# interaction-lab-uh/STROTSS-tensorflow

Measured on AMD Instinct MI355X. Metric: optimisation_steps_per_sec_1024px_pair, higher is better.
Workload: dtype f32; 1 GPU; 1024px content/style pair, 1024x1024 scale of the coarse-to-fine pyramid, 1024 samples x D=2179, VGG16 (seeded He-normal weights), RMSprop pixel update; scale_px=1024, samples=1024, parallelism=single GPU, tap_adjoint=deterministic (planned, sorted scatter)

## Files before the change

strotss-tensorflow_amd/csrc/gemm.hip:

```cpp
#include <stdlib.h>

#include "internal.h"
#include "mfma_pipe.h"
#include "mfma_x3.h"

namespace {

template <int BM, int BN, bool AKC, bool BKC>
__device__ __forceinline__ void gemm_mainloop(const float* __restrict__ A, int lda, int M,
                                              const float* __restrict__ B, int ldb, int N, int K,
                                              int m0, int n0, float* ldsA, float* ldsB,
                                              f32x16 (&acc)[BM / 64][BN / 64]) {
  f32x4 ra[BM / 32], rb[BN / 32];
  auto load = [&](int k0) {
    if constexpr (AKC) gload_kc<BM>(ra, A, lda, m0, M, k0); else gload_rc<BM>(ra, A, lda, m0, M, k0);
    if constexpr (BKC) gload_kc<BN>(rb, B, ldb, n0, N, k0); else gload_rc<BN>(rb, B, ldb, n0, N, k0);
  };
  load(0);
  for (int k0 = 0; k0 < K; k0 += 32) {
    __syncthreads();
    if constexpr (AKC) lds_store_kc<BM>(ldsA, ra); else lds_store_rc<BM>(ldsA, ra);
    if constexpr (BKC) lds_store_kc<BN>(ldsB, rb); else lds_store_rc<BN>(ldsB, rb);
    __syncthreads();
    if (k0 + 32 < K) load(k0 + 32);
// ... 224 lines not shown
  }
  return v;
}

template <int BM, int BN, class Epi>
int launch_pipe(const float* A, int lda, int M, long long strideA, const float* B, int ldb, int N,
                long long strideB, int K, int batch, Epi epi, hipStream_t s) {
  dim3 grid((unsigned)cdiv(N, BN) * cdiv(M, BM) * batch);
  if constexpr (BM == 128) {
    if (gemm_waves() == 8) {
      using Cfg = PipeCfg<BM, BN, (BN == 128 ? 2 : 4), (BN == 128 ? 4 : 2)>;
      hipLaunchKernelGGL((gemm_kc_pipe_kernel<Cfg, Epi>), grid, dim3(Cfg::NT), 0, s, A, lda, M, strideA, B, ldb, N,
                         strideB, K, epi);
      ST_LAUNCH_RET();
    }
  }
  {
    using Cfg = PipeCfg<BM, BN, 2, 2>;
    hipLaunchKernelGGL((gemm_kc_pipe_kernel<Cfg, Epi>), grid, dim3(Cfg::NT), 0, s, A, lda, M, strideA, B, ldb, N,
                       strideB, K, epi);
  }
  ST_LAUNCH_RET();
}

template <int BM, int BN, bool AKC, bool BKC, class Epi>
int launch(const float* A, int lda, int M, const float* B, int ldb, int N, int K, Epi epi,
           hipStream_t s) {
  dim3 grid(cdiv(N, BN), cdiv(M, BM));
  hipLaunchKernelGGL((gemm_kernel<BM, BN, AKC, BKC, Epi>), grid, dim3(256), 0, s, A, lda, M, B, ldb, N,
                     K, epi);
  ST_LAUNCH_RET();
}

}

int st_cosine_distance(const float* x, const float* rx, int nx, const float* y, const float* ry, int ny,
                       int ld, float* C, int ldc, hipStream_t s) {
  EpiCosDist e{rx, ry, C, ldc, nx, ny, (x == y && rx == ry && nx == ny) ? 1 : 0};
  return launch_pipe<64, 64>(x, ld, nx, 0, y, ld, ny, 0, ld, 1, e, s);
}

int st_l2_distance(const float* x, const float* xs, int nx, const float* y, const float* ys, int ny, int ld, int d,
                   float* C, int ldc, hipStream_t s) {
  EpiL2Dist e{xs, ys, C, ldc, nx, ny, (float)d};
  return launch_pipe<64, 64>(x, ld, nx, 0, y, ld, ny, 0, ld, 1, e, s);
}

int st_remd_cost(const float* x, const float* rx, const float* sx, int nx, const float* y, const float* ry, const float* sy,
                 int ny, int ld, int d, int metric, float* C, float* S, int ldc, hipStream_t s) {
  EpiRemdCost e{rx, ry, sx, sy, C, S, ldc, nx, ny, (float)d, metric};
  return launch_pipe<64, 64>(x, ld, nx, 0, y, ld, ny, 0, ld, 1, e, s);
}

int st_gram_tn(const float* A, int krows, int ld, float alpha, float* C, hipStream_t s) {
  EpiScaleStore e{C, ld, ld, ld, alpha, 0};
  return launch<64, 64, false, false>(A, ld, ld, A, ld, ld, krows, e, s);
}

int st_moment_fwd_gemm(const float* cy, int krows, int ld, const float* Sx, float* T, float inv_n,
                       float* partial, int* n_partial, hipStream_t s) {
  EpiMomentFwd e{Sx, T, ld, ld, ld, inv_n, partial};
  *n_partial = cdiv(ld, 64) * cdiv(ld, 64);
  return launch<64, 64, false, false>(cy, ld, ld, cy, ld, ld, krows, e, s);
}

int st_moment_bwd_gemm(const float* cy, int n, int ld, const float* T, float alpha, const float* bias,
                       float bias_scale, float* dY, hipStream_t s) {
  EpiAxpbyBias e{dY, ld, n, ld, alpha, bias, bias_scale};
  return launch_pipe<64, 64>(cy, ld, n, 0, T, ld, ld, 0, ld, 1, e, s);
}

int st_selfsim_bwd_gemm(const float* Mq, int ldm, int kpad, const float* bmat, const float* x, const float* r,
                        const float* q, int n, int ld, float g, float* dx, hipStream_t s) {
  EpiSelfsimBwd e{x, r, q, dx, ld, n, ld, g};
  return launch<64, 64, true, false>(Mq, ldm, n, bmat, ld, ld, kpad, e, s);
}

int st_gemm_nt_batched(const float* A, int lda, long long strideA, const float* B, int ldb, long long strideB,
                       float* C, int ldc, long long strideC, int M, int N, int K, int batch, hipStream_t s) {
  EpiScaleStore e{C, ldc, M, N, 1.0f, strideC};
  const long long t128 = (long long)cdiv(M, 128) * cdiv(N, 128);
  if (t128 * batch >= 512 && N % 128 == 0) {
    static int split = -1;
    if (split < 0) { const char* env = getenv("STROTSS_GEMM_TAIL_SPLIT"); split = env ? atoi(env) : 1; }
    const long long slots = 512, total = t128 * batch;
    const long long rem = total % slots;
    if (split && total > slots && rem != 0 && rem * 2 <= slots && slots % t128 == 0) {
      const int tail = (int)(rem / t128), head = batch - tail;
      int rc = launch_pipe<128, 128>(A, lda, M, strideA, B, ldb, N, strideB, K, head, e, s);
      if (rc != 0) return rc;
      EpiScaleStore e2{C + (long long)head * strideC, ldc, M, N, 1.0f, strideC};
      return launch_pipe<128, 64>(A + (long long)head * strideA, lda, M, strideA, B + (long long)head * strideB, ldb, N,
                                  strideB, K, tail, e2, s);
    }
    return launch_pipe<128, 128>(A, lda, M, strideA, B, ldb, N, strideB, K, batch, e, s);
  }
  const long long t64 = (long long)cdiv(M, 128) * cdiv(N, 64);
  if (t64 * batch >= 512) {
    static int split = -1;
    if (split < 0) { const char* env = getenv("STROTSS_GEMM_TAIL_SPLIT"); split = env ? atoi(env) : 1; }
    const long long slots = 512, total = t64 * batch, rem = total % slots;
    if (split && total > slots && rem != 0 && rem * 2 <= slots && slots % t64 == 0) {
      const int tail = (int)(rem / t64), head = batch - tail;
      int rc = launch_pipe<128, 64>(A, lda, M, strideA, B, ldb, N, strideB, K, head, e, s);
      if (rc != 0) return rc;
      EpiScaleStore e2{C + (long long)head * strideC, ldc, M, N, 1.0f, strideC};
      return launch_pipe<64, 64>(A + (long long)head * strideA, lda, M, strideA, B + (long long)head * strideB, ldb, N,
                                 strideB, K, tail, e2, s);
    }
    return launch_pipe<128, 64>(A, lda, M, strideA, B, ldb, N, strideB, K, batch, e, s);
  }
  return launch_pipe<64, 64>(A, lda, M, strideA, B, ldb, N, strideB, K, batch, e, s);
}

int st_x3_split_rows(const float* x, int rows, int ld, int K, long long stride_in, void* panels, int batch,
                     hipStream_t s) {
  const size_t total = (size_t)rows * (K >> 2);
  hipLaunchKernelGGL(x3_split_rows_kernel, dim3((unsigned)min((size_t)2048, (total + 255) / 256), batch), dim3(256), 0, s,
                     x, rows, ld, K, stride_in, (__bf16*)panels, (long long)3 * rows * K);
  ST_LAUNCH_RET();
}

struct EpiScaleStoreX3 : EpiScaleStore, X3NoPrefetch<EpiScaleStoreX3> {
  using EpiScaleStore::apply;
  using X3NoPrefetch<EpiScaleStoreX3>::apply;
};
struct X3NoMirror {
  template <class Epi, class Pre, class Acc, class Map>
  __device__ __forceinline__ void operator()(const Epi&, Pre&, float*, int, int, int, int, Acc&, const Map&) const {}
};
template <class Cfg>
struct X3Mirror {
  template <class Epi, class Pre, class Acc, class Map>
  __device__ __forceinline__ void operator()(const Epi& epi, Pre&, float* tile, int m0, int n0, int M, int N, Acc& acc,
                                             const Map& map) const {
    mirror_tile<Cfg::BM, Cfg::BN, Cfg::NT, true>(epi, tile, m0, n0, M, N, [&](auto put) {
#pragma unroll
      for (int im = 0; im < Cfg::T; ++im)
#pragma unroll
        for (int in = 0; in < Cfg::T; ++in)
#pragma unroll
          for (int reg = 0; reg < 16; ++reg) {
            const int r = m0 + map.row(im, reg), c = n0 + map.colof(in);
            put(r, c, (r < M && c < N) ? epi.value(r, c, acc[im][in][reg]) : 0.f);
          }
    });
  }
};

static bool x3_k16_enabled() {
  static const bool k16 = [] { const char* v = getenv("STROTSS_X3_K16"); return !v || atoi(v) != 0; }();
  return k16;
}
int st_gemm_x3_batched(const void* A, const void* B, float* C, int ldc, long long strideC, int M, int N, int K,
                       int batch, hipStream_t s, long min_tiles128) {
  EpiScaleStoreX3 e{{C, ldc, M, N, 1.0f, strideC}, {}};
  if ((long)cdiv(N, 128) * cdiv(M, 128) * batch >= min_tiles128 && x3_k16_enabled()) {
    using Cfg = X3CfgK16<3>;
    dim3 grid((unsigned)cdiv(N, 128) * cdiv(M, 128) * batch);
    hipLaunchKernelGGL((gemm_x3_kernel<Cfg, EpiScaleStoreX3, X3NoMirror>), grid, dim3(Cfg::NT), 0, s, (const __bf16*)A, M,
                       (long long)3 * M * K, (const __bf16*)B, N, (long long)3 * N * K, K, e, X3NoMirror{});
  } else if ((long)cdiv(N, 128) * cdiv(M, 128) * batch >= min_tiles128) {
    using Cfg = X3Cfg<128>;
    dim3 grid((unsigned)cdiv(N, 128) * cdiv(M, 128) * batch);
    hipLaunchKernelGGL((gemm_x3_kernel<Cfg, EpiScaleStoreX3, X3NoMirror>), grid, dim3(Cfg::NT), 0, s, (const __bf16*)A, M,
                       (long long)3 * M * K, (const __bf16*)B, N, (long long)3 * N * K, K, e, X3NoMirror{});
  } else {
    using Cfg = X3Cfg<64>;
    dim3 grid((unsigned)cdiv(N, 64) * cdiv(M, 64) * batch);
    hipLaunchKernelGGL((gemm_x3_kernel<Cfg, EpiScaleStoreX3, X3NoMirror>), grid, dim3(Cfg::NT), 0, s, (const __bf16*)A, M,
                       (long long)3 * M * K, (const __bf16*)B, N, (long long)3 * N * K, K, e, X3NoMirror{});
  }
  ST_LAUNCH_RET();
}

bool st_gemm_x3_f32a_ok(int M, int N, int batch, long min_tiles128) {
  return (long)cdiv(N, 128) * cdiv(M, 128) * batch >= min_tiles128 && x3_k16_enabled();
}
int st_gemm_x3_batched_f32a(const float* A, const void* B, float* C, int ldc, long long strideC, int M, int N, int K,
                            int batch, hipStream_t s, long min_tiles128) {
  if (!st_gemm_x3_f32a_ok(M, N, batch, min_tiles128)) return STROTSS_EINVAL;
  EpiScaleStoreX3 e{{C, ldc, M, N, 1.0f, strideC}, {}};
  using Cfg = X3CfgK16<3, true>;
  dim3 grid((unsigned)cdiv(N, 128) * cdiv(M, 128) * batch);
  hipLaunchKernelGGL((gemm_x3_kernel<Cfg, EpiScaleStoreX3, X3NoMirror>), grid, dim3(Cfg::NT), 0, s, A, M, (long long)M * K,
                     (const __bf16*)B, N, (long long)3 * N * K, K, e, X3NoMirror{});
  ST_LAUNCH_RET();
}

struct EpiSelfsimBwdX3 : EpiSelfsimBwd {
  template <int T> struct Pre { float dx0[T][T][16], x0[T][T][16], ri[T][16], qi[T][16]; };
  template <class P> __device__ __forceinline__ void prefetch(P& p, int im, int in, int reg, int row, int c) const {
    const int rr = min(row, M - 1);
    const size_t o = (size_t)rr * ld + min(c, N - 1);
    p.dx0[im][in][reg] = dx[o];
    p.x0[im][in][reg] = x[o];
    if (in == 0) { p.ri[im][reg] = r[rr]; p.qi[im][reg] = q[rr]; }
  }
  template <class P> __device__ __forceinline__ float apply(P& p, int im, int in, int reg, int row, int c, float v) const {
    const float ri = p.ri[im][reg];
    const float out = p.dx0[im][in][reg] + g * ri * (v - p.x0[im][in][reg] * ri * p.qi[im][reg]);
    if (row < M && c < N) dx[(size_t)row * ld + c] = out;
    return 0.f;
  }
};
struct EpiAxpbyBiasX3 : EpiAxpbyBias {
  template <int T> struct Pre { float c0[T][T][16], b[T]; };
  template <class P> __device__ __forceinline__ void prefetch(P& p, int im, int in, int reg, int r, int c) const {
    p.c0[im][in][reg] = C[(size_t)min(r, M - 1) * ldc + min(c, N - 1)];
    if (im == 0 && reg == 0) p.b[in] = bias[min(c, N - 1)];
  }
  template <class P> __device__ __forceinline__ float apply(P& p, int im, int in, int reg, int r, int c, float v) const {
    const float out = p.c0[im][in][reg] + alpha * v + bias_scale * p.b[in];
    if (r < M && c < N) C[(size_t)r * ldc + c] = out;
    return 0.f;
  }
};
struct EpiMomentFwdX3 {
  static constexpr bool SYMM = true;
  static constexpr int symm = 1;
  const float* Sx; __bf16* Tp; int ld; int M, N; float inv_n; float* partial;
  unsigned first_block = 0;
  __device__ __forceinline__ void set_batch(int) {}
  template <int T> struct Pre { float sx[T][T][16]; };
  template <class P> __device__ __forceinline__ void prefetch(P& p, int im, int in, int reg, int r, int c) const {
    p.sx[im][in][reg] = Sx[(size_t)min(r, M - 1) * ld + min(c, N - 1)];
  }
  template <class P> __device__ __forceinline__ float apply(P& p, int im, int in, int reg, int r, int c, float v) const {
    const float a = fabsf(v * inv_n - p.sx[im][in][reg]);
    const float w = (r < M && c < N && r <= c) ? (r == c ? 1.f : 2.f) : 0.f;
    return w * a;
  }
  __device__ __forceinline__ void finish(float* red, float local) const {
    const float s = block_sum_256(local, red);
    if (threadIdx.x == 0) partial[blockIdx.x - first_block] = s;
  }
};
template <class Cfg>
struct X3MomentStore {
  template <class Pre, class Acc, class Map>
  __device__ __forceinline__ void operator()(const EpiMomentFwdX3& epi, Pre& pre, float* tile, int m0, int n0, int M, int N,
                                             Acc& acc, const Map& map) const {
    constexpr int B = Cfg::BM, LD = B + 1;
    __syncthreads();
#pragma unroll
    for (int im = 0; im < Cfg::T; ++im)
#pragma unroll
      for (int in = 0; in < Cfg::T; ++in)
#pragma unroll
        for (int reg = 0; reg < 16; ++reg) {
          const int r = map.row(im, reg), c = map.colof(in);
          tile[r * LD + c] = signf(acc[im][in][reg] * epi.inv_n - pre.sx[im][in][reg]);
        }
    __syncthreads();
    const bool diag = n0 == m0;
    if (diag) {
      for (int i = threadIdx.x; i < B * B; i += Cfg::NT) {
        const int r = i / B, c = i - r * B;
        if (r > c) tile[r * LD + c] = tile[c * LD + r];
      }
      __syncthreads();
    }
    auto put8 = [&](int row, int k0, const float (&v)[8]) {
      bf16x8 o;
#pragma unroll
      for (int q = 0; q < 8; ++q) o[q] = (__bf16)v[q];
      *reinterpret_cast<bf16x8*>(epi.Tp + ((size_t)(k0 >> 5) * epi.ld + row) * 32 + (k0 & 31)) = o;
    };
    for (int i = threadIdx.x; i < B * (B / 8); i += Cfg::NT) {
      const int r = i / (B / 8), c8 = (i - r * (B / 8)) * 8;
      if (m0 + r >= M || n0 + c8 >= N) continue;
      float v[8];
#pragma unroll
      for (int q = 0; q < 8; ++q) v[q] = tile[r * LD + c8 + q];
      put8(m0 + r, n0 + c8, v);
    }
    if (!diag) {
      for (int i = threadIdx.x; i < B * (B / 8); i += Cfg::NT) {
        const int c = i % B, r8 = (i / B) * 8;
        if (n0 + c >= N || m0 + r8 >= M) continue;
        float v[8];
#pragma unroll
        for (int q = 0; q < 8; ++q) v[q] = tile[(r8 + q) * LD + c];
        put8(n0 + c, m0 + r8, v);
      }
    }
  }
};

struct EpiSymScaleX3 : X3NoPrefetch<EpiSymScaleX3> {
  using X3NoPrefetch<EpiSymScaleX3>::apply;
  static constexpr bool SYMM = true;
  static constexpr int symm = 1;
  float* C; int ld; int M, N; float alpha;
  __device__ __forceinline__ void set_batch(int) {}
  __device__ __forceinline__ float value(int, int, float v) const { return alpha * v; }
  __device__ __forceinline__ float apply(int r, int c, float v) const {
    if (r < M && c < N && r <= c) C[(size_t)r * ld + c] = alpha * v;
    return 0.f;
  }
  __device__ __forceinline__ void mirror(int r, int c, float val) const { C[(size_t)r * ld + c] = val; }
  __device__ __forceinline__ void finish(float*, float) const {}
};
int st_gram_tn_x3(const void* Pt, int npad, int ld, float alpha, float* C, hipStream_t s) {
  using Cfg = X3CfgK16<3>;
  EpiSymScaleX3 e{{}, C, ld, ld, ld, alpha};
  const int g = cdiv(ld, 128);
  hipLaunchKernelGGL((gemm_x3_kernel<Cfg, EpiSymScaleX3, X3Mirror<Cfg>>), dim3(g * (g + 1) / 2), dim3(Cfg::NT), 0, s,
                     (const __bf16*)Pt, ld, 0LL, (const __bf16*)Pt, ld, 0LL, npad, e, X3Mirror<Cfg>{});
  ST_LAUNCH_RET();
}

int st_moment_fwd_x3(const void* Pt, int npad, int ld, const float* Sx, void* Tp, float inv_n, float* partial,
                     int* n_partial, hipStream_t s) {
  using Cfg = X3CfgK16<3>;
  EpiMomentFwdX3 e{Sx, (__bf16*)Tp, ld, ld, ld, inv_n, partial, 0u};
  const int g = cdiv(ld, 128);
  *n_partial = g * (g + 1) / 2;
  hipLaunchKernelGGL((gemm_x3_kernel<Cfg, EpiMomentFwdX3, X3MomentStore<Cfg>>), dim3(g * (g + 1) / 2), dim3(Cfg::NT), 0, s,
                     (const __bf16*)Pt, ld, 0LL, (const __bf16*)Pt, ld, 0LL, npad, e, X3MomentStore<Cfg>{});
  ST_LAUNCH_RET();
}

int st_loss_forward_group_x3(const void* Pt, int npad, int ld, const float* Sx, void* Tp, float inv_n, float* partial,
                             int* n_partial,
                             const void* xp, const float* rp, int n, long long pstride, long long rstride, float* Dx,
                             int ldc, long long dstride,
                             const void* xs, const float* rs, int ns, float* Ct, int ldt, hipStream_t s) {
  using CM = X3CfgK16<3>;
  using CC = X3Cfg<64>;
  const unsigned gm = cdiv(ld, 128), nm = gm * (gm + 1) / 2;
  const unsigned g = cdiv(n, 64), nc = g * (g + 1) / 2 * 2;
  const unsigned gs = cdiv(ns, 64), nr = g * gs;
  *n_partial = (int)nm;
  X3Problem<EpiMomentFwdX3> p0{(const __bf16*)Pt, ld, 0LL, (const __bf16*)Pt, ld, 0LL, npad,
                               EpiMomentFwdX3{Sx, (__bf16*)Tp, ld, ld, ld, inv_n, partial, 0u}, 0, 0, nm};
  X3Problem<EpiCosDistX3> p1{(const __bf16*)xp, n, pstride, (const __bf16*)xp, n, pstride, ld,
                             EpiCosDistX3{{rp, rp, Dx, ldc, n, n, 1}, {}, rstride, dstride}, 0, 0, nc};
  int bh = 0, bw = 0;
// ... 118 lines not shown
```

strotss-tensorflow_amd/csrc/mfma_x3.h:

```cpp
#pragma once
#include <type_traits>

#include "mfma_pipe.h"

typedef __bf16 bf16x8 __attribute__((ext_vector_type(8)));
typedef __bf16 bf16x4 __attribute__((ext_vector_type(4)));
typedef unsigned int u32x4 __attribute__((ext_vector_type(4)));

struct Split3 { bf16x4 h, m, l; };
__device__ __forceinline__ Split3 split3(const f32x4 x) {
  Split3 s;
#pragma unroll
  for (int k = 0; k < 4; ++k) {
    const __bf16 h = (__bf16)x[k];
    const float r1 = x[k] - (float)h;
    const __bf16 m = (__bf16)r1;
    const float r2 = r1 - (float)m;
    s.h[k] = h; s.m[k] = m; s.l[k] = (__bf16)r2;
  }
  return s;
}

__host__ __device__ __forceinline__ size_t x3_panel_elems(size_t rows, size_t K) { return 3 * rows * K; }
__device__ __forceinline__ void x3_store4(__bf16* base, size_t rows, size_t row, int k0, const f32x4 v) {
  const Split3 s = split3(v);
  const size_t o = ((size_t)(k0 >> 5) * 3 * rows + row) * 32 + (k0 & 31);
  *reinterpret_cast<bf16x4*>(base + o) = s.h;
  *reinterpret_cast<bf16x4*>(base + o + rows * 32) = s.m;
  *reinterpret_cast<bf16x4*>(base + o + 2 * rows * 32) = s.l;
}

template <int B_, int NPB_ = 3>
struct X3Cfg {
  static_assert(B_ == 128 || B_ == 64, "x3 main loop: 128 x 128 or 64 x 64 tiles");
  static_assert(NPB_ == 3 || (NPB_ == 1 && B_ == 128), "single-plane B: 128 x 128 tiles only");
  static constexpr int NPB = NPB_, NPROD = NPB_ == 3 ? 6 : 3;
  static constexpr int BM = B_, BN = B_, WM = 2, WN = 2, NT = 256;
  static constexpr int T = B_ / 64;
  static constexpr int TM = T, TN = T;
  static constexpr int PL = B_ * 64;
  static constexpr int STAGE = (3 + NPB_) * PL;
  static constexpr int LDS_BYTES = 3 * STAGE;
  static constexpr int G = B_ / 64;
  static constexpr int NP = (3 + NPB_) * G;
  static constexpr bool K16 = false, AF32 = false;
};

#define X3_WAIT_VM(n) asm volatile("s_waitcnt vmcnt(" #n ")" ::: "memory")

template <int G, int NPL = 3>
struct X3Operand {
  const char* base;
  unsigned off[G];
  unsigned plane;
  unsigned cur;
  __device__ __forceinline__ X3Operand(const __bf16* p, int rows, int row0) {
    const int lane = threadIdx.x & 63, wave = __builtin_amdgcn_readfirstlane(threadIdx.x >> 6);
    base = reinterpret_cast<const char*>(p);
    plane = (unsigned)rows * 64u;
    cur = 0;
    const int chunk = (lane & 3) ^ ((lane >> 4) & 3);
#pragma unroll
    for (int g = 0; g < G; ++g) {
      const int row = min(row0 + (G * wave + g) * 16 + (lane >> 2), rows - 1);
      off[g] = (unsigned)row * 64u + (unsigned)chunk * 16u;
    }
  }
  __device__ __forceinline__ void dma(int pl, int g, unsigned char* lds_dst) const {
    const char* src = base + (size_t)(cur + pl * plane) + off[g];
    __builtin_amdgcn_global_load_lds((const __attribute__((address_space(1))) void*)src,
                                     (__attribute__((address_space(3))) void*)lds_dst, 16, 0, 0);
  }
  __device__ __forceinline__ void advance() { cur += NPL * plane; }
};

template <class Cfg>
__device__ __forceinline__ void x3_mainloop(unsigned char* lds, int steps, X3Operand<Cfg::G, 3>& oa,
                                            X3Operand<Cfg::G, Cfg::NPB>& ob, f32x16 (&acc)[Cfg::T][Cfg::T]) {
  constexpr int PL = Cfg::PL, STAGE = Cfg::STAGE, T = Cfg::T, G = Cfg::G, NP = Cfg::NP, HALF = Cfg::BM / 2;
  constexpr int NPB = Cfg::NPB, NPROD = Cfg::NPROD;
  const int t = threadIdx.x, lane = t & 63, wave = __builtin_amdgcn_readfirstlane(t >> 6);
  const int wm = wave >> 1, wn = wave & 1, l31 = lane & 31, hh = lane >> 5;
  auto dma_piece = [&](int j, unsigned char* stage) {
#ifdef X3_ABL_NO_DMA
    return;
#endif
    const int pl = j / G, g = j % G;
    unsigned char* dst = stage + pl * PL + (G * wave + g) * 1024;
    if (pl < 3) oa.dma(pl, g, dst); else ob.dma(pl - 3, g, dst);
  };
  auto dma_tile = [&](unsigned char* stage) {
#pragma unroll
    for (int j = 0; j < NP; ++j) dma_piece(j, stage);
    oa.advance(); ob.advance();
  };
  auto wait_one_tile_in_flight = [&]() {
    if constexpr (NP == 12) X3_WAIT_VM(12); else if constexpr (NP == 8) X3_WAIT_VM(8); else X3_WAIT_VM(6);
  };
  const int f = (l31 >> 2) & 3;
  const int a_rd = (wm * HALF + l31) * 64 + ((hh ^ f) << 4);
  const int b_rd = 3 * PL + (wn * HALF + l31) * 64 + ((hh ^ f) << 4);
  bf16x8 fa[2][3][T], fb[2][NPB][T];
  auto read_frags = [&](const unsigned char* stage, int kc, int slot) {
#ifdef X3_ABL_NO_FRAG
    if (stage != lds) return;
#endif
    const unsigned char* pa = stage + (a_rd ^ (kc << 5));
    const unsigned char* pb = stage + (b_rd ^ (kc << 5));
#pragma unroll
    for (int p = 0; p < 3; ++p) {
#pragma unroll
      for (int i = 0; i < T; ++i) {
        fa[slot][p][i] = *reinterpret_cast<const bf16x8*>(pa + p * PL + i * 2048);
        if (p < NPB) fb[slot][p][i] = *reinterpret_cast<const bf16x8*>(pb + p * PL + i * 2048);
      }
    }
  };
  constexpr int PA[6] = {2, NPB == 3 ? 0 : 1, NPB == 3 ? 1 : 0, 1, 0, 0};
  constexpr int PB[6] = {0, NPB == 3 ? 2 : 0, NPB == 3 ? 1 : 0, 0, 1, 0};
  constexpr int STRIDE = NPROD * T * T / NP;
  static_assert(STRIDE >= 1, "more DMA pieces than MFMAs in a k-chunk");

  unsigned char* s_cur = lds;
  unsigned char* s_nxt = lds + STAGE;
  unsigned char* s_nn = lds + 2 * STAGE;
  dma_tile(s_cur);
  if (steps > 1) { dma_tile(s_nxt); wait_one_tile_in_flight(); } else { X3_WAIT_VM(0); }
  __builtin_amdgcn_s_barrier();
  read_frags(s_cur, 0, 0);

  auto kstep = [&](auto mode_tag) {
    constexpr int MODE = decltype(mode_tag)::value;
#pragma unroll
    for (int c = 0; c < 2; ++c) {
#pragma unroll
      for (int q = 0; q < NPROD; ++q) {
        if (c == 0 && q == 1) {
          __builtin_amdgcn_sched_barrier(0);
          read_frags(s_cur, 1, 1);
          __builtin_amdgcn_sched_barrier(0);
        }
#pragma unroll
        for (int im = 0; im < T; ++im) {
#pragma unroll
          for (int in_ = 0; in_ < T; ++in_) {
#ifndef X3_ABL_NO_MFMA
            acc[im][in_] = __builtin_amdgcn_mfma_f32_32x32x16_bf16(fa[c][PA[q]][im], fb[c][PB[q]][in_], acc[im][in_], 0, 0, 0);
#else
            acc[im][in_][0] += (float)fa[c][PA[q]][im][0] + (float)fb[c][PB[q]][in_][0];
#endif
            const int done = (q * T + im) * T + in_ + 1;
            if (MODE == 2 && c == 0 && done % STRIDE == 0 && done / STRIDE <= NP) {
              __builtin_amdgcn_sched_barrier(0);
              dma_piece(done / STRIDE - 1, s_nn);
              __builtin_amdgcn_sched_barrier(0);
            }
          }
        }
        if (c == 1 && q == 0 && MODE != 0) {
          __builtin_amdgcn_sched_barrier(0);
          if (MODE == 2) wait_one_tile_in_flight(); else X3_WAIT_VM(0);
          asm volatile("s_waitcnt lgkmcnt(0)" ::: "memory");
#ifndef X3_ABL_NO_BARRIER
          __builtin_amdgcn_s_barrier();
#endif
          asm volatile("" ::: "memory");
          read_frags(s_nxt, 0, 0);
          __builtin_amdgcn_sched_barrier(0);
        }
      }
    }
    if (MODE == 2) { oa.advance(); ob.advance(); }
    unsigned char* tmp = s_cur; s_cur = s_nxt; s_nxt = s_nn; s_nn = tmp;
  };
  int s = 0;
  for (; s + 2 < steps; ++s) kstep(std::integral_constant<int, 2>{});
  if (steps > 1) kstep(std::integral_constant<int, 1>{});
  kstep(std::integral_constant<int, 0>{});
}

template <int NPB_ = 3, bool AF32_ = false, int WQ_ = AF32_ ? 1 : 3>
struct X3CfgK16 {
  static_assert(NPB_ == 3, "K16 ring: three B planes");
  static_assert(WQ_ >= 0 && WQ_ <= 4, "K16 ring: the wait needs at least one product group after it");
  static constexpr int NPB = NPB_, NPROD = 6;
  static constexpr bool AF32 = AF32_;
  static constexpr int WQ = WQ_;
  static constexpr int BM = 128, BN = 128, WM = 2, WN = 2, NT = 256;
  static constexpr int T = 2, TM = 2, TN = 2;
  static constexpr int PL = 128 * 32;
  static constexpr int NPA = AF32_ ? 2 : 3;
  static constexpr int ABYTES = NPA * PL;
  static constexpr int STAGE = ABYTES + 3 * PL;
  static constexpr int LDS_BYTES = 3 * STAGE;
  static constexpr int G = 1, NP = NPA + 3;
  static constexpr bool K16 = true;
};

struct X3OperandK16 {
  const char* base;
  unsigned off;
  unsigned plane;
  unsigned cur;
  __device__ __forceinline__ X3OperandK16(const __bf16* p, int rows, int row0) {
    const int lane = threadIdx.x & 63, wave = __builtin_amdgcn_readfirstlane(threadIdx.x >> 6);
    base = reinterpret_cast<const char*>(p);
    plane = (unsigned)rows * 64u;
    cur = 0;
    const int row = min(row0 + wave * 32 + (lane >> 1), rows - 1);
    off = (unsigned)row * 64u + (unsigned)((lane & 1) ^ ((lane >> 4) & 1)) * 16u;
  }
  __device__ __forceinline__ void dma(int pl, unsigned char* lds_dst) const {
    const char* src = base + (size_t)(cur + pl * plane) + off;
    __builtin_amdgcn_global_load_lds((const __attribute__((address_space(1))) void*)src,
                                     (__attribute__((address_space(3))) void*)lds_dst, 16, 0, 0);
  }
  __device__ __forceinline__ void advance(int half) { cur += half ? 3u * plane - 32u : 32u; }
};

struct X3OperandK16F32 {
  const char* base;
  unsigned off[2];
  unsigned kblk;
  unsigned cur;
  __device__ __forceinline__ X3OperandK16F32(const float* p, int rows, int row0) {
    const int lane = threadIdx.x & 63, wave = __builtin_amdgcn_readfirstlane(threadIdx.x >> 6);
    base = reinterpret_cast<const char*>(p);
    kblk = (unsigned)rows * 128u;
    cur = 0;
    const int chunk = (lane & 3) ^ ((lane >> 4) & 3);
#pragma unroll
    for (int g = 0; g < 2; ++g) {
      const int row = min(row0 + wave * 32 + g * 16 + (lane >> 2), rows - 1);
      off[g] = (unsigned)row * 128u + (unsigned)chunk * 16u;
    }
  }
  __device__ __forceinline__ void dma(int g, unsigned char* lds_dst) const {
    const char* src = base + (size_t)cur + off[g];
    __builtin_amdgcn_global_load_lds((const __attribute__((address_space(1))) void*)src,
                                     (__attribute__((address_space(3))) void*)lds_dst, 16, 0, 0);
  }
  __device__ __forceinline__ void advance(int half) { cur += half ? kblk - 64u : 64u; }
};

__device__ __forceinline__ void x3_f32_store4(float* base, size_t rows, size_t row, int k0, const f32x4 v) {
  *reinterpret_cast<f32x4*>(base + ((size_t)(k0 >> 5) * rows + row) * 32 + (k0 & 31)) = v;
}

__device__ __forceinline__ void x3_split8(const f32x4 lo, const f32x4 hi, bf16x8& h, bf16x8& m, bf16x8& l) {
  const Split3 a = split3(lo), b = split3(hi);
  h = __builtin_shufflevector(a.h, b.h, 0, 1, 2, 3, 4, 5, 6, 7);
  m = __builtin_shufflevector(a.m, b.m, 0, 1, 2, 3, 4, 5, 6, 7);
  l = __builtin_shufflevector(a.l, b.l, 0, 1, 2, 3, 4, 5, 6, 7);
}

template <class Cfg> struct X3Ops {
  using A = std::conditional_t<Cfg::K16, std::conditional_t<Cfg::AF32, X3OperandK16F32, X3OperandK16>, X3Operand<Cfg::G, 3>>;
  using B = std::conditional_t<Cfg::K16, X3OperandK16, X3Operand<Cfg::G, Cfg::NPB>>;
  using AT = std::conditional_t<Cfg::AF32, float, __bf16>;
};

template <class Cfg, class OA>
__device__ __forceinline__ void x3_k16_prologue(unsigned char* lds, OA& oa, X3OperandK16& ob) {
#ifndef X3_ABL_NO_DMA
  const int wave = __builtin_amdgcn_readfirstlane(threadIdx.x >> 6);
#pragma unroll
  for (int h = 0; h < 2; ++h) {
    unsigned char* stage = lds + h * Cfg::STAGE;
#pragma unroll
    for (int j = 0; j < Cfg::NP; ++j) {
      if (j >= Cfg::NPA) ob.dma(j - Cfg::NPA, stage + Cfg::ABYTES + (j - Cfg::NPA) * Cfg::PL + wave * 1024);
      else if constexpr (Cfg::AF32) oa.dma(j, stage + wave * 2048 + j * 1024);
      else oa.dma(j, stage + j * Cfg::PL + wave * 1024);
    }
    oa.advance(h); ob.advance(h);
  }
#endif
}

template <class Cfg, class OA>
__device__ __forceinline__ void x3_mainloop_k16(unsigned char* lds, int steps, OA& oa, X3OperandK16& ob,
                                                f32x16 (&acc)[2][2]) {
  constexpr int PL = Cfg::PL, STAGE = Cfg::STAGE, NPA = Cfg::NPA, NP = Cfg::NP, WQ = Cfg::WQ;
  constexpr bool AF32 = Cfg::AF32;
  static_assert(NP == 5 || NP == 6, "K16 ring: 5 or 6 DMA pieces per wave and step");
  const int t = threadIdx.x, lane = t & 63, wave = __builtin_amdgcn_readfirstlane(t >> 6);
  const int wm = wave >> 1, wn = wave & 1, l31 = lane & 31, hh = lane >> 5;
  auto dma_piece = [&](int j, unsigned char* stage) {
#ifdef X3_ABL_NO_DMA
    return;
#endif
    if (j >= NPA) ob.dma(j - NPA, stage + Cfg::ABYTES + (j - NPA) * PL + wave * 1024);
    else if constexpr (AF32) oa.dma(j, stage + wave * 2048 + j * 1024);
    else oa.dma(j, stage + j * PL + wave * 1024);
  };
  constexpr int IN_FLIGHT = 4 * (WQ + 1) < NP ? 4 * (WQ + 1) : NP;
  auto wait_next_tile = [&]() {
    if constexpr (IN_FLIGHT == 6) X3_WAIT_VM(6); else if constexpr (IN_FLIGHT == 5) X3_WAIT_VM(5); else X3_WAIT_VM(4);
  };
  int half = 0;
  const int sw = (hh ^ ((l31 >> 3) & 1)) << 4;
  const int a_rd = (wm * 64 + l31) * 32 + sw;
  const int b_rd = Cfg::ABYTES + (wn * 64 + l31) * 32 + sw;
  const int af = (l31 >> 2) & 3;
  const int a_rd0 = (wm * 64 + l31) * 64 + (((2 * hh) ^ af) << 4), a_rd1 = (wm * 64 + l31) * 64 + (((2 * hh + 1) ^ af) << 4);
  bf16x8 fa[2][3][2], fb[2][3][2];
  f32x4 ra[2][2];
  auto read_frags = [&](const unsigned char* stage, int slot) {
#ifdef X3_ABL_NO_FRAG
    if (stage != lds) return;
#endif
#pragma unroll
    for (int i = 0; i < 2; ++i) {
      if constexpr (AF32) {
        ra[i][0] = *reinterpret_cast<const f32x4*>(stage + a_rd0 + i * 2048);
        ra[i][1] = *reinterpret_cast<const f32x4*>(stage + a_rd1 + i * 2048);
      }
#pragma unroll
      for (int p = 0; p < 3; ++p) {
        if constexpr (!AF32) fa[slot][p][i] = *reinterpret_cast<const bf16x8*>(stage + a_rd + p * PL + i * 1024);
        fb[slot][p][i] = *reinterpret_cast<const bf16x8*>(stage + b_rd + p * PL + i * 1024);
      }
    }
  };
  auto split_a = [&](int slot) {
    if constexpr (AF32) {
#pragma unroll
      for (int i = 0; i < 2; ++i) x3_split8(ra[i][0], ra[i][1], fa[slot][0][i], fa[slot][1][i], fa[slot][2][i]);
    }
  };
  constexpr int PA[6] = {2, 0, 1, 1, 0, 0};
  constexpr int PB[6] = {0, 2, 1, 0, 1, 0};

  unsigned char* s_cur = lds;
  unsigned char* s_nxt = lds + STAGE;
  unsigned char* s_nn = lds + 2 * STAGE;
  if constexpr (NP == 6) X3_WAIT_VM(6); else X3_WAIT_VM(5);
  __builtin_amdgcn_s_barrier();
  read_frags(s_cur, 0);
  split_a(0);

  auto kstep = [&](auto mode_tag, auto slot_tag) {
    constexpr int MODE = decltype(mode_tag)::value, SLOT = decltype(slot_tag)::value;
#pragma unroll
    for (int q = 0; q < 6; ++q) {
#pragma unroll
      for (int im = 0; im < 2; ++im) {
#pragma unroll
        for (int in_ = 0; in_ < 2; ++in_) {
#ifndef X3_ABL_NO_MFMA
          acc[im][in_] = __builtin_amdgcn_mfma_f32_32x32x16_bf16(fa[SLOT][PA[q]][im], fb[SLOT][PB[q]][in_], acc[im][in_], 0, 0, 0);
#else
          acc[im][in_][0] += (float)fa[SLOT][PA[q]][im][0] + (float)fb[SLOT][PB[q]][in_][0];
#endif
          const int done = (q * 2 + im) * 2 + in_ + 1;
          if (MODE == 2 && done <= NP) {
            __builtin_amdgcn_sched_barrier(0);
            dma_piece(done - 1, s_nn);
            __builtin_amdgcn_sched_barrier(0);
          }
        }
      }
      if (q == WQ && MODE != 0) {
        __builtin_amdgcn_sched_barrier(0);
        if (MODE == 2) wait_next_tile(); else X3_WAIT_VM(0);
        asm volatile("s_waitcnt lgkmcnt(0)" ::: "memory");
#ifndef X3_ABL_NO_BARRIER
        __builtin_amdgcn_s_barrier();
#endif
        asm volatile("" ::: "memory");
        read_frags(s_nxt, SLOT ^ 1);
        __builtin_amdgcn_sched_barrier(0);
        split_a(SLOT ^ 1);
      }
    }
    if (MODE == 2) { oa.advance(half); ob.advance(half); half ^= 1; }
    unsigned char* tmp = s_cur; s_cur = s_nxt; s_nxt = s_nn; s_nn = tmp;
  };
  using I0 = std::integral_constant<int, 0>; using I1 = std::integral_constant<int, 1>; using I2 = std::integral_constant<int, 2>;
  int s = 0;
  for (; s + 3 < steps; s += 2) { kstep(I2{}, I0{}); kstep(I2{}, I1{}); }
  kstep(I1{}, I0{});
  kstep(I0{}, I1{});
}

template <class D>
struct X3NoPrefetch {
  template <int T> struct Pre {};
  template <class P> __device__ __forceinline__ void prefetch(P&, int, int, int, int, int) const {}
  template <class P> __device__ __forceinline__ float apply(P&, int, int, int, int r, int c, float v) const {
    return static_cast<const D*>(this)->apply(r, c, v);
  }
};

template <class Cfg, class Epi, class Mirror>
__device__ __forceinline__ void gemm_x3_tile(unsigned char* lds, unsigned bid, unsigned nblk,
                                             const typename X3Ops<Cfg>::AT* __restrict__ A, int M,
                                             long long strideA, const __bf16* __restrict__ B, int N, long long strideB, int K,
                                             const Epi& epi_in, const Mirror& mirror, int xbh, int xbw) {
  Epi epi = epi_in;
  const unsigned gx = (N + Cfg::BN - 1) / Cfg::BN, gy = (M + Cfg::BM - 1) / Cfg::BM;
  unsigned tile = xcd_swizzle(bid, nblk);
  unsigned bz = 0;
  int m0, n0;
  bool tri = false;
  if constexpr (Epi::SYMM) tri = epi.symm != 0;
  if (tri) {
    const unsigned ntri = gx * (gx + 1) / 2;
    bz = tile / ntri;
    tile -= bz * ntri;
    unsigned i = 0, len = gx;
    while (tile >= len) { tile -= len; --len; ++i; }
    m0 = i * Cfg::BM; n0 = (i + tile) * Cfg::BN;
  } else {
    bz = tile / (gx * gy);
    const unsigned rem = tile - bz * (gx * gy);
    if (xbh > 0) {
      const unsigned per = (unsigned)(xbh * xbw), blk = rem / per, in = rem - blk * per;
      const unsigned bpr = gx / (unsigned)xbw;
      const unsigned ty = (blk / bpr) * xbh + in / xbw, tx = (blk % bpr) * xbw + in % xbw;
      m0 = ty * Cfg::BM; n0 = tx * Cfg::BN;
    } else {
      m0 = (rem / gx) * Cfg::BM; n0 = (rem % gx) * Cfg::BN;
    }
  }
  epi.set_batch(bz);
  typename X3Ops<Cfg>::A oa(A + (long long)bz * strideA, M, m0);
  typename X3Ops<Cfg>::B ob(B + (long long)bz * strideB, N, n0);
  f32x16 acc[Cfg::T][Cfg::T];
#pragma unroll
  for (int i = 0; i < Cfg::T; ++i)
#pragma unroll
    for (int j = 0; j < Cfg::T; ++j)
#pragma unroll
      for (int r = 0; r < 16; ++r) acc[i][j][r] = 0.f;
  PipeAccMap<Cfg> map;
  typename Epi::template Pre<Cfg::T> pre;
#pragma unroll
  for (int im = 0; im < Cfg::T; ++im)
#pragma unroll
    for (int in = 0; in < Cfg::T; ++in)
#pragma unroll
      for (int reg = 0; reg < 16; ++reg)
        epi.prefetch(pre, im, in, reg, m0 + map.row(im, reg), n0 + map.colof(in));
  if constexpr (Cfg::K16) { x3_k16_prologue<Cfg>(lds, oa, ob); x3_mainloop_k16<Cfg>(lds, K >> 4, oa, ob, acc); }
  else x3_mainloop<Cfg>(lds, K >> 5, oa, ob, acc);
  float local = 0.f;
#pragma unroll
  for (int im = 0; im < Cfg::T; ++im)
#pragma unroll
    for (int in = 0; in < Cfg::T; ++in)
#pragma unroll
      for (int reg = 0; reg < 16; ++reg)
        local += epi.apply(pre, im, in, reg, m0 + map.row(im, reg), n0 + map.colof(in), acc[im][in][reg]);
  if constexpr (Epi::SYMM) {
    static_assert(!Epi::SYMM || Cfg::LDS_BYTES >= Cfg::BM * (Cfg::BN + 1) * 4, "mirror tile");
    if (epi.symm && n0 >= m0) mirror(epi, pre, reinterpret_cast<float*>(lds), m0, n0, M, N, acc, map);
  }
  __syncthreads();
  epi.finish(reinterpret_cast<float*>(lds), local);
}

template <class Cfg, class Epi, class Mirror>
__global__ __launch_bounds__(Cfg::NT) void gemm_x3_kernel(const typename X3Ops<Cfg>::AT* __restrict__ A, int M, long long strideA,
                                                          const __bf16* __restrict__ B, int N, long long strideB,
                                                          int K, Epi epi, Mirror mirror, int xbh = 0, int xbw = 0) {
  __shared__ __attribute__((aligned(1024))) unsigned char lds[Cfg::LDS_BYTES];
  gemm_x3_tile<Cfg, Epi, Mirror>(lds, blockIdx.x, gridDim.x, A, M, strideA, B, N, strideB, K, epi, mirror, xbh, xbw);
}

template <class Epi>
struct X3Problem {
  const __bf16* A; int M; long long strideA;
  const __bf16* B; int N; long long strideB;
  int K; Epi epi; int xbh, xbw;
  unsigned n;
};
__host__ __device__ __forceinline__ unsigned x3_pad8(unsigned n) { return (n + 7u) & ~7u; }
template <class C0, class E0, class M0, class C1, class E1, class M1, class C2, class E2, class M2>
__global__ __launch_bounds__(256) void gemm_x3_group3_kernel(X3Problem<E0> p0, X3Problem<E1> p1, X3Problem<E2> p2) {
  static_assert(C0::NT == 256 && C1::NT == 256 && C2::NT == 256, "grouped x3 launch: 256-thread workgroups");
  constexpr int L01 = C0::LDS_BYTES > C1::LDS_BYTES ? C0::LDS_BYTES : C1::LDS_BYTES;
  constexpr int LDSB = L01 > C2::LDS_BYTES ? L01 : C2::LDS_BYTES;
  __shared__ __attribute__((aligned(1024))) unsigned char lds[LDSB];
  unsigned b = blockIdx.x;
  if (b < x3_pad8(p0.n)) {
    if (b < p0.n) { M0 m; gemm_x3_tile<C0, E0, M0>(lds, b, p0.n, p0.A, p0.M, p0.strideA, p0.B, p0.N, p0.strideB, p0.K, p0.epi, m, p0.xbh, p0.xbw); }
    return;
  }
  b -= x3_pad8(p0.n);
  if (b < x3_pad8(p1.n)) {
    if (b < p1.n) { M1 m; gemm_x3_tile<C1, E1, M1>(lds, b, p1.n, p1.A, p1.M, p1.strideA, p1.B, p1.N, p1.strideB, p1.K, p1.epi, m, p1.xbh, p1.xbw); }
    return;
  }
  b -= x3_pad8(p1.n);
  if (b < p2.n) { M2 m; gemm_x3_tile<C2, E2, M2>(lds, b, p2.n, p2.A, p2.M, p2.strideA, p2.B, p2.N, p2.strideB, p2.K, p2.epi, m, p2.xbh, p2.xbw); }
}

#define X3_MAX_SET 4
template <class Epi>
struct X3ProblemSet {
  X3Problem<Epi> q[X3_MAX_SET];
  int count;
};
template <class C0, class E0, class M0, class C1, class E1, class M1, class C2, class E2, class M2>
__global__ __launch_bounds__(256) void gemm_x3_group_set_kernel(X3Problem<E0> p0, X3Problem<E1> p1, X3ProblemSet<E2> ps) {
  static_assert(C0::NT == 256 && C1::NT == 256 && C2::NT == 256, "grouped x3 launch: 256-thread workgroups");
  constexpr int L01 = C0::LDS_BYTES > C1::LDS_BYTES ? C0::LDS_BYTES : C1::LDS_BYTES;
  constexpr int LDSB = L01 > C2::LDS_BYTES ? L01 : C2::LDS_BYTES;
  __shared__ __attribute__((aligned(1024))) unsigned char lds[LDSB];
  unsigned b = blockIdx.x;
  if (b < x3_pad8(p0.n)) {
    if (b < p0.n) { M0 m; gemm_x3_tile<C0, E0, M0>(lds, b, p0.n, p0.A, p0.M, p0.strideA, p0.B, p0.N, p0.strideB, p0.K, p0.epi, m, p0.xbh, p0.xbw); }
    return;
  }
  b -= x3_pad8(p0.n);
  if (b < x3_pad8(p1.n)) {
    if (b < p1.n) { M1 m; gemm_x3_tile<C1, E1, M1>(lds, b, p1.n, p1.A, p1.M, p1.strideA, p1.B, p1.N, p1.strideB, p1.K, p1.epi, m, p1.xbh, p1.xbw); }
    return;
  }
  b -= x3_pad8(p1.n);
  int k = 0;
  while (k < ps.count && k < X3_MAX_SET && b >= x3_pad8(ps.q[k].n)) { b -= x3_pad8(ps.q[k].n); ++k; }
  if (k >= ps.count || k >= X3_MAX_SET) return;
  const X3Problem<E2>& p = ps.q[k];
  if (b < p.n) { M2 m; gemm_x3_tile<C2, E2, M2>(lds, b, p.n, p.A, p.M, p.strideA, p.B, p.N, p.strideB, p.K, p.epi, m, p.xbh, p.xbw); }
}

static __global__ __launch_bounds__(256) void x3_split_rows_kernel(const float* __restrict__ x, int rows, int ld, int K,
                                                            long long stride_in, __bf16* __restrict__ out,
                                                            long long stride_out) {
  x += (long long)blockIdx.y * stride_in;
  out += (long long)blockIdx.y * stride_out;
  const size_t total = (size_t)rows * (K >> 2);
  for (size_t e = (size_t)blockIdx.x * 256 + threadIdx.x; e < total; e += (size_t)gridDim.x * 256) {
    const int k4 = (int)(e & 7);
    const size_t rr = e >> 3;
    const int row = (int)(rr % rows), kb = (int)(rr / rows);
    const int k0 = kb * 32 + k4 * 4;
    x3_store4(out, rows, row, k0, *reinterpret_cast<const f32x4*>(x + (size_t)row * ld + k0));
  }
}
```

Baseline: 232.6 steps/s.

## Use two-stage LDS ring for f32-A x3 conv GEMM to raise occupancy

Adds a two-stage variant of the K16 x3 GEMM ring. The f32-A conv path now uses it by default, and the old three-stage version stays behind an env var. With two stages the next tile's DMA is issued after the barrier into the buffer just consumed, not spread across the MFMA groups, and the LDS footprint shrinks so launch bounds can request 3 workgroups per CU. The aim is more concurrent workgroups to hide latency, at the cost of less overlap between loads and compute inside each workgroup and more register pressure. It also adds a debug ablation macro that skips the prologue DMA.

New measurement: 233.7 steps/s, median of 6. About the same (+0.4%).

```diff
diff --git a/strotss-tensorflow_amd/csrc/gemm.hip b/strotss-tensorflow_amd/csrc/gemm.hip
--- a/strotss-tensorflow_amd/csrc/gemm.hip
+++ b/strotss-tensorflow_amd/csrc/gemm.hip
@@ -400,6 +400,10 @@
   static const bool k16 = [] { const char* v = getenv("STROTSS_X3_K16"); return !v || atoi(v) != 0; }();
   return k16;
 }
+static bool x3_conv_ring3() {
+  static const bool on = [] { const char* v = getenv("STROTSS_X3_CONV_RING3"); return v && atoi(v) != 0; }();
+  return on;
+}
 int st_gemm_x3_batched(const void* A, const void* B, float* C, int ldc, long long strideC, int M, int N, int K,
                        int batch, hipStream_t s, long min_tiles128) {
   EpiScaleStoreX3 e{{C, ldc, M, N, 1.0f, strideC}, {}};
@@ -429,10 +433,16 @@
                             int batch, hipStream_t s, long min_tiles128) {
   if (!st_gemm_x3_f32a_ok(M, N, batch, min_tiles128)) return STROTSS_EINVAL;
   EpiScaleStoreX3 e{{C, ldc, M, N, 1.0f, strideC}, {}};
-  using Cfg = X3CfgK16<3, true>;
   dim3 grid((unsigned)cdiv(N, 128) * cdiv(M, 128) * batch);
-  hipLaunchKernelGGL((gemm_x3_kernel<Cfg, EpiScaleStoreX3, X3NoMirror>), grid, dim3(Cfg::NT), 0, s, A, M, (long long)M * K,
-                     (const __bf16*)B, N, (long long)3 * N * K, K, e, X3NoMirror{});
+  if (x3_conv_ring3()) {
+    using Cfg = X3CfgK16<3, true>;
+    hipLaunchKernelGGL((gemm_x3_kernel<Cfg, EpiScaleStoreX3, X3NoMirror>), grid, dim3(Cfg::NT), 0, s, A, M, (long long)M * K,
+                       (const __bf16*)B, N, (long long)3 * N * K, K, e, X3NoMirror{});
+  } else {
+    using Cfg = X3CfgK16<3, true, 1, 2>;
+    hipLaunchKernelGGL((gemm_x3_kernel<Cfg, EpiScaleStoreX3, X3NoMirror>), grid, dim3(Cfg::NT), 0, s, A, M, (long long)M * K,
+                       (const __bf16*)B, N, (long long)3 * N * K, K, e, X3NoMirror{});
+  }
   ST_LAUNCH_RET();
 }
 
diff --git a/strotss-tensorflow_amd/csrc/mfma_x3.h b/strotss-tensorflow_amd/csrc/mfma_x3.h
--- a/strotss-tensorflow_amd/csrc/mfma_x3.h
+++ b/strotss-tensorflow_amd/csrc/mfma_x3.h
@@ -40,6 +40,7 @@
   static constexpr int TM = T, TN = T;
   static constexpr int PL = B_ * 64;
   static constexpr int STAGE = (3 + NPB_) * PL;
+  static constexpr int MIN_WAVES = 1;
   static constexpr int LDS_BYTES = 3 * STAGE;
   static constexpr int G = B_ / 64;
   static constexpr int NP = (3 + NPB_) * G;
@@ -124,8 +125,13 @@
   unsigned char* s_cur = lds;
   unsigned char* s_nxt = lds + STAGE;
   unsigned char* s_nn = lds + 2 * STAGE;
+#ifdef X3_ABL_NO_PROLOGUE
+  oa.advance(); ob.advance();
+  if (steps > 1) { oa.advance(); ob.advance(); }
+#else
   dma_tile(s_cur);
   if (steps > 1) { dma_tile(s_nxt); wait_one_tile_in_flight(); } else { X3_WAIT_VM(0); }
+#endif
   __builtin_amdgcn_s_barrier();
   read_frags(s_cur, 0, 0);
 
@@ -179,9 +185,12 @@
   kstep(std::integral_constant<int, 0>{});
 }
 
-template <int NPB_ = 3, bool AF32_ = false, int WQ_ = AF32_ ? 1 : 3>
+template <int NPB_ = 3, bool AF32_ = false, int WQ_ = AF32_ ? 1 : 3, int NS_ = 3>
 struct X3CfgK16 {
   static_assert(NPB_ == 3, "K16 ring: three B planes");
+  static_assert(NS_ == 2 || NS_ == 3, "K16 ring: two or three stages");
+  static constexpr int NS = NS_;
+  static constexpr int MIN_WAVES = NS_ == 2 ? 3 : 1;
   static_assert(WQ_ >= 0 && WQ_ <= 4, "K16 ring: the wait needs at least one product group after it");
   static constexpr int NPB = NPB_, NPROD = 6;
   static constexpr bool AF32 = AF32_;
@@ -192,7 +201,7 @@
   static constexpr int NPA = AF32_ ? 2 : 3;
   static constexpr int ABYTES = NPA * PL;
   static constexpr int STAGE = ABYTES + 3 * PL;
-  static constexpr int LDS_BYTES = 3 * STAGE;
+  static constexpr int LDS_BYTES = NS_ * STAGE;
   static constexpr int G = 1, NP = NPA + 3;
   static constexpr bool K16 = true;
 };
@@ -262,7 +271,9 @@
 
 template <class Cfg, class OA>
 __device__ __forceinline__ void x3_k16_prologue(unsigned char* lds, OA& oa, X3OperandK16& ob) {
-#ifndef X3_ABL_NO_DMA
+#if defined(X3_ABL_NO_PROLOGUE)
+  oa.advance(0); ob.advance(0); oa.advance(1); ob.advance(1);
+#elif !defined(X3_ABL_NO_DMA)
   const int wave = __builtin_amdgcn_readfirstlane(threadIdx.x >> 6);
 #pragma unroll
   for (int h = 0; h < 2; ++h) {
@@ -281,7 +292,7 @@
 template <class Cfg, class OA>
 __device__ __forceinline__ void x3_mainloop_k16(unsigned char* lds, int steps, OA& oa, X3OperandK16& ob,
                                                 f32x16 (&acc)[2][2]) {
-  constexpr int PL = Cfg::PL, STAGE = Cfg::STAGE, NPA = Cfg::NPA, NP = Cfg::NP, WQ = Cfg::WQ;
+  constexpr int PL = Cfg::PL, STAGE = Cfg::STAGE, NPA = Cfg::NPA, NP = Cfg::NP, WQ = Cfg::WQ, NS = Cfg::NS;
   constexpr bool AF32 = Cfg::AF32;
   static_assert(NP == 5 || NP == 6, "K16 ring: 5 or 6 DMA pieces per wave and step");
   const int t = threadIdx.x, lane = t & 63, wave = __builtin_amdgcn_readfirstlane(t >> 6);
@@ -334,7 +345,7 @@
 
   unsigned char* s_cur = lds;
   unsigned char* s_nxt = lds + STAGE;
-  unsigned char* s_nn = lds + 2 * STAGE;
+  unsigned char* s_nn = lds + (NS - 1) * STAGE;
   if constexpr (NP == 6) X3_WAIT_VM(6); else X3_WAIT_VM(5);
   __builtin_amdgcn_s_barrier();
   read_frags(s_cur, 0);
@@ -354,7 +365,7 @@
           acc[im][in_][0] += (float)fa[SLOT][PA[q]][im][0] + (float)fb[SLOT][PB[q]][in_][0];
 #endif
           const int done = (q * 2 + im) * 2 + in_ + 1;
-          if (MODE == 2 && done <= NP) {
+          if (NS == 3 && MODE == 2 && done <= NP) {
             __builtin_amdgcn_sched_barrier(0);
             dma_piece(done - 1, s_nn);
             __builtin_amdgcn_sched_barrier(0);
@@ -363,7 +374,7 @@
       }
       if (q == WQ && MODE != 0) {
         __builtin_amdgcn_sched_barrier(0);
-        if (MODE == 2) wait_next_tile(); else X3_WAIT_VM(0);
+        if (MODE == 2 && NS == 3) wait_next_tile(); else X3_WAIT_VM(0);
         asm volatile("s_waitcnt lgkmcnt(0)" ::: "memory");
 #ifndef X3_ABL_NO_BARRIER
         __builtin_amdgcn_s_barrier();
@@ -371,11 +382,17 @@
         asm volatile("" ::: "memory");
         read_frags(s_nxt, SLOT ^ 1);
         __builtin_amdgcn_sched_barrier(0);
+        if (NS == 2 && MODE == 2) {
+#pragma unroll
+          for (int j = 0; j < NP; ++j) dma_piece(j, s_cur);
+          __builtin_amdgcn_sched_barrier(0);
+        }
         split_a(SLOT ^ 1);
       }
     }
     if (MODE == 2) { oa.advance(half); ob.advance(half); half ^= 1; }
-    unsigned char* tmp = s_cur; s_cur = s_nxt; s_nxt = s_nn; s_nn = tmp;
+    if constexpr (NS == 3) { unsigned char* tmp = s_cur; s_cur = s_nxt; s_nxt = s_nn; s_nn = tmp; }
+    else { unsigned char* tmp = s_cur; s_cur = s_nxt; s_nxt = tmp; }
   };
   using I0 = std::integral_constant<int, 0>; using I1 = std::integral_constant<int, 1>; using I2 = std::integral_constant<int, 2>;
   int s = 0;
@@ -462,7 +479,7 @@
 }
 
 template <class Cfg, class Epi, class Mirror>
-__global__ __launch_bounds__(Cfg::NT) void gemm_x3_kernel(const typename X3Ops<Cfg>::AT* __restrict__ A, int M, long long strideA,
+__global__ __launch_bounds__(Cfg::NT, Cfg::MIN_WAVES) void gemm_x3_kernel(const typename X3Ops<Cfg>::AT* __restrict__ A, int M, long long strideA,
                                                           const __bf16* __restrict__ B, int N, long long strideB,
                                                           int K, Epi epi, Mirror mirror, int xbh = 0, int xbw = 0) {
   __shared__ __attribute__((aligned(1024))) unsigned char lds[Cfg::LDS_BYTES];
```
